# mfkiwl/msckf_stereo_c

Hardware: AMD Instinct MI355X
Metric: stereo frames/sec/node on EuRoC-shape input; ATE RMSE vs CPU ref (higher is better)
Workload: dtype f64

## Files before the change

### msckf_stereo_c_amd/csrc/hip/fe_kernels.hip

```cpp
#include <stdlib.h>
#include <mutex>
#include "fe_device.h"

__device__ __forceinline__ int reflect101(int i, int n) {
    if (n == 1) return 0;
    while (i < 0 || i >= n) { i = (i < 0) ? -i : 2 * (n - 1) - i; }
    return i;
}

#define P3_TW 16
#define P3_TH 8
struct Pyr3Job { const uint8_t *src; uint8_t *d1, *d2, *d3; int w0, h0; };

namespace {
constexpr int P3_R2H = 2 * P3_TH + 4, P3_R1H = 2 * P3_R2H + 4, P3_R0H = 2 * P3_R1H + 4;
constexpr int P3_P2W = 2 * P3_TW + 8, P3_P1W = 2 * (2 * P3_TW + 4) + 8;
constexpr int P3_P1S = P3_P1W + 8, P3_P2S = P3_P2W + 8;
typedef uint32_t __attribute__((aligned(1))) pd_u32u;

__device__ __forceinline__ uint2 pd_h4(uint32_t w0, uint32_t w1, uint32_t w2) {
    const int b0 = w0 & 255u, b1 = (w0 >> 8) & 255u, b2 = (w0 >> 16) & 255u, b3 = w0 >> 24, b4 = w1 & 255u, b5 = (w1 >> 8) & 255u,
              b6 = (w1 >> 16) & 255u, b7 = w1 >> 24, b8 = w2 & 255u, b9 = (w2 >> 8) & 255u, b10 = (w2 >> 16) & 255u;
    const uint32_t h0 = (uint32_t)(b0 + 4 * b1 + 6 * b2 + 4 * b3 + b4), h1 = (uint32_t)(b2 + 4 * b3 + 6 * b4 + 4 * b5 + b6);
    const uint32_t h2 = (uint32_t)(b4 + 4 * b5 + 6 * b6 + 4 * b7 + b8), h3 = (uint32_t)(b6 + 4 * b7 + 6 * b8 + 4 * b9 + b10);
    uint2 o; o.x = h0 | (h1 << 16); o.y = h2 | (h3 << 16);
    return o;
}
__device__ __forceinline__ uint32_t pd_v4(uint2 r0, uint2 r1, uint2 r2, uint2 r3, uint2 r4) {
    const uint32_t lo = (r0.x + r4.x) + 4u * (r1.x + r3.x) + 6u * r2.x + 0x00800080u;
    const uint32_t hi = (r0.y + r4.y) + 4u * (r1.y + r3.y) + 6u * r2.y + 0x00800080u;
    return ((lo >> 8) & 255u) | ((lo >> 24) << 8) | (((hi >> 8) & 255u) << 16) | ((hi >> 24) << 24);
}
__device__ __forceinline__ void pd_store4(uint8_t *row, int x, int w, uint32_t px) {
    if (x + 3 < w) *reinterpret_cast<pd_u32u *>(row + x) = px;
    else for (int k = 0; x + k < w; ++k) row[x + k] = (uint8_t)(px >> (8 * k));
}
__device__ __forceinline__ void pd_fill_halo(uint8_t *plane, int stride, int rows, int cols, int y_base, int x_base, int w, int h, int tid) {
    for (int i = tid; i < 4 * rows; i += 256) {
        const int r = i >> 2, q = i & 3;
        const int x = q < 2 ? q - 2 : w + q - 2, y = y_base + r;
        const int c = x - x_base;
        if (c < 0 || c >= cols || y < -2 || y > h + 1) continue;
        const int ys = reflect101(y, h) - y_base, xs = reflect101(x, w) - x_base;
        if (ys < 0 || ys >= rows || xs < 0 || xs >= cols) continue;
        plane[r * stride + 4 + c] = plane[ys * stride + 4 + xs];
    }
    for (int i = tid; i < 4 * cols; i += 256) {
        const int q = i / cols, c = i - q * cols;
        const int y = q < 2 ? q - 2 : h + q - 2, x = x_base + c;
        const int r = y - y_base;
        if (r < 0 || r >= rows || x < 0 || x >= w) continue;
        const int ys = reflect101(y, h) - y_base;
        if (ys < 0 || ys >= rows) continue;
        plane[r * stride + 4 + c] = plane[ys * stride + 4 + c];
    }
}
}

__global__ __launch_bounds__(256) void k_pyr_down3(const Pyr3Job *jobs, int n_jobs, int tiles_x, int tiles_y) {
    const int tiles = tiles_x * tiles_y;
    const int bx = blockIdx.x & 7, bq = blockIdx.x >> 3;
    const int ji = bx + 8 * (bq / tiles), tile = bq - (bq / tiles) * tiles;
    if (ji >= n_jobs) return;
    const Pyr3Job job = jobs[ji];
    const int w0 = job.w0, h0 = job.h0, w1 = (w0 + 1) >> 1, h1 = (h0 + 1) >> 1, w2 = (w1 + 1) >> 1, h2 = (h1 + 1) >> 1, w3 = (w2 + 1) >> 1, h3 = (h2 + 1) >> 1;
    const int ty = tile / tiles_x, tx = tile - ty * tiles_x;
    const int x3_0 = tx * P3_TW, y3_0 = ty * P3_TH;
    if (x3_0 >= w3 || y3_0 >= h3) return;
    __shared__ __attribute__((aligned(16))) uint16_t s_h0[P3_R0H][P3_P1W];
    __shared__ __attribute__((aligned(16))) uint8_t s_p1[P3_R1H][P3_P1S];
    __shared__ __attribute__((aligned(16))) uint16_t s_h1[P3_R1H][P3_P2W];
    __shared__ __attribute__((aligned(16))) uint8_t s_p2[P3_R2H][P3_P2S];
    __shared__ __attribute__((aligned(16))) uint16_t s_h2[P3_R2H][P3_TW];
    const int tid = threadIdx.x;
    const int x1b = 4 * x3_0 - 8, y1b = 4 * y3_0 - 6, y0b = 8 * y3_0 - 14;
    const int x2b = 2 * x3_0 - 4, y2b = 2 * y3_0 - 2;
    {
        const int pa = max(0, -y0b), pb = min(P3_R0H, h0 - y0b);
        constexpr int NG = P3_P1W / 4;
        int ga = (1 - x1b + 3) >> 2; ga = ga < 0 ? 0 : ga;
        int gb = min(min((w1 - 4 - x1b) >> 2, (w0 - 10 - 2 * x1b) >> 3) + 1, NG);
        if (w1 - 4 - x1b < 0 || w0 - 10 - 2 * x1b < 0) gb = 0;
        if (gb < ga) gb = ga;
        const int ng = gb - ga, n_fast = (pb - pa) * ng;
        const unsigned inv = ng > 0 ? (65536u + (unsigned)ng - 1u) / (unsigned)ng : 0u;
        constexpr int MAXIT = (P3_R0H * NG + 255) / 256;
        uint32_t la[MAXIT], lb[MAXIT], lc[MAXIT];
#pragma unroll
        for (int it = 0; it < MAXIT; ++it) {
            const int idx = tid + 256 * it;
            la[it] = lb[it] = lc[it] = 0u;
            if (idx < n_fast) {
                const int pr = (int)(((unsigned)idx * inv) >> 16), g = ga + idx - pr * ng, p = pa + pr;
                const uint8_t *q = job.src + (size_t)(y0b + p) * w0 + (2 * (x1b + 4 * g) - 2);
                la[it] = *reinterpret_cast<const pd_u32u *>(q); lb[it] = *reinterpret_cast<const pd_u32u *>(q + 4); lc[it] = *reinterpret_cast<const pd_u32u *>(q + 8);
            }
        }
#pragma unroll
        for (int it = 0; it < MAXIT; ++it) {
            const int idx = tid + 256 * it;
            if (idx < n_fast) {
                const int pr = (int)(((unsigned)idx * inv) >> 16), g = ga + idx - pr * ng, p = pa + pr;
                *reinterpret_cast<uint2 *>(&s_h0[p][4 * g]) = pd_h4(la[it], lb[it], lc[it]);
            }
        }
        const int n_edge = NG - ng, n_slow = (pb - pa) * n_edge;
        for (int idx = tid; idx < n_slow; idx += 256) {
            const int pr = idx / n_edge, e = idx - pr * n_edge, g = e < ga ? e : gb + (e - ga), p = pa + pr;
            const uint8_t *row = job.src + (size_t)(y0b + p) * w0;
#pragma unroll
            for (int j = 0; j < 4; ++j) {
                const int x1 = x1b + 4 * g + j;
                if (x1 < 0 || x1 >= w1) continue;
                const int c = 2 * x1;
                s_h0[p][4 * g + j] = (uint16_t)(row[reflect101(c - 2, w0)] + 4 * row[reflect101(c - 1, w0)] + 6 * row[reflect101(c, w0)] +
                                                4 * row[reflect101(c + 1, w0)] + row[reflect101(c + 2, w0)]);
            }
        }
    }
    __syncthreads();
    {
        const int ra = max(0, -y1b), rb = min(P3_R1H, h1 - y1b);
        constexpr int NG = P3_P1W / 4;
        const int n = (rb - ra) * NG;
        for (int idx = tid; idx < n; idx += 256) {
            const int rr = idx / NG, g = idx - rr * NG, r = ra + rr;
            const int y1 = y1b + r, x1 = x1b + 4 * g;
            if (x1 + 3 < 0 || x1 >= w1) continue;
            uint2 v[5];
#pragma unroll
            for (int k = 0; k < 5; ++k) {
                const int p = min(max(reflect101(2 * y1 - 2 + k, h0) - y0b, 0), P3_R0H - 1);
                v[k] = *reinterpret_cast<const uint2 *>(&s_h0[p][4 * g]);
            }
            const uint32_t px = pd_v4(v[0], v[1], v[2], v[3], v[4]);
            *reinterpret_cast<uint32_t *>(&s_p1[r][4 + 4 * g]) = px;
            if (r >= 6 && r < 6 + 4 * P3_TH && g >= 2 && g < 2 + P3_TW && x1 >= 0) pd_store4(job.d1 + (size_t)y1 * w1, x1, w1, px);
        }
    }
    __syncthreads();
    const bool edge1 = x1b < 0 || y1b < 0 || x1b + P3_P1W > w1 || y1b + P3_R1H > h1;
    if (edge1) { pd_fill_halo(&s_p1[0][0], P3_P1S, P3_R1H, P3_P1W, y1b, x1b, w1, h1, tid); __syncthreads(); }
    {
        constexpr int NG = P3_P2W / 4;
        const int ra = max(0, -2 - y1b), rb = min(P3_R1H, h1 + 2 - y1b);
        const int n = (rb - ra) * NG;
        for (int idx = tid; idx < n; idx += 256) {
            const int rr = idx / NG, g = idx - rr * NG, r = ra + rr;
            const uint32_t *q = reinterpret_cast<const uint32_t *>(&s_p1[r][8 * g]);
            const uint32_t d0 = q[0], d1 = q[1], d2 = q[2], d3 = q[3];
            *reinterpret_cast<uint2 *>(&s_h1[r][4 * g]) = pd_h4(__builtin_amdgcn_alignbyte(d1, d0, 2), __builtin_amdgcn_alignbyte(d2, d1, 2), __builtin_amdgcn_alignbyte(d3, d2, 2));
        }
    }
    __syncthreads();
    {
        constexpr int NG = P3_P2W / 4;
        const int ra = max(0, -y2b), rb = min(P3_R2H, h2 - y2b);
        const int n = (rb - ra) * NG;
        for (int idx = tid; idx < n; idx += 256) {
            const int rr = idx / NG, g = idx - rr * NG, r = ra + rr;
            const int y2 = y2b + r, x2 = x2b + 4 * g;
            if (x2 + 3 < 0 || x2 >= w2) continue;
            uint2 v[5];
#pragma unroll
            for (int k = 0; k < 5; ++k) v[k] = *reinterpret_cast<const uint2 *>(&s_h1[2 * r + k][4 * g]);
            const uint32_t px = pd_v4(v[0], v[1], v[2], v[3], v[4]);
            *reinterpret_cast<uint32_t *>(&s_p2[r][4 + 4 * g]) = px;
            if (r >= 2 && r < 2 + 2 * P3_TH && g >= 1 && g < 1 + P3_TW / 2 && x2 >= 0) pd_store4(job.d2 + (size_t)y2 * w2, x2, w2, px);
        }
    }
    __syncthreads();
    const bool edge2 = x2b < 0 || y2b < 0 || x2b + P3_P2W > w2 || y2b + P3_R2H > h2;
    if (edge2) { pd_fill_halo(&s_p2[0][0], P3_P2S, P3_R2H, P3_P2W, y2b, x2b, w2, h2, tid); __syncthreads(); }
    {
        constexpr int NG = P3_TW / 4;
        const int ra = max(0, -2 - y2b), rb = min(P3_R2H, h2 + 2 - y2b);
        const int n = (rb - ra) * NG;
        for (int idx = tid; idx < n; idx += 256) {
            const int rr = idx / NG, g = idx - rr * NG, r = ra + rr;
            const uint32_t *q = reinterpret_cast<const uint32_t *>(&s_p2[r][4 + 8 * g]);
            const uint32_t d0 = q[0], d1 = q[1], d2 = q[2], d3 = q[3];
            *reinterpret_cast<uint2 *>(&s_h2[r][4 * g]) = pd_h4(__builtin_amdgcn_alignbyte(d1, d0, 2), __builtin_amdgcn_alignbyte(d2, d1, 2), __builtin_amdgcn_alignbyte(d3, d2, 2));
        }
    }
    __syncthreads();
    {
        constexpr int NG = P3_TW / 4;
        const int rb = min(P3_TH, h3 - y3_0);
        const int n = rb * NG;
        for (int idx = tid; idx < n; idx += 256) {
            const int r = idx / NG, g = idx - r * NG;
            const int x3 = x3_0 + 4 * g;
            if (x3 >= w3) continue;
            uint2 v[5];
#pragma unroll
            for (int k = 0; k < 5; ++k) v[k] = *reinterpret_cast<const uint2 *>(&s_h2[2 * r + k][4 * g]);
            pd_store4(job.d3 + (size_t)(y3_0 + r) * w3, x3, w3, pd_v4(v[0], v[1], v[2], v[3], v[4]));
        }
    }
}

extern "C" void fe_launch_pyr_down3(const Pyr3Job *jobs_dev, int n_jobs, int max_w0, int max_h0, hipStream_t st) {
    const int w3 = (((max_w0 + 1) / 2 + 1) / 2 + 1) / 2, h3 = (((max_h0 + 1) / 2 + 1) / 2 + 1) / 2;
    const int tiles_x = (w3 + P3_TW - 1) / P3_TW, tiles_y = (h3 + P3_TH - 1) / P3_TH;
    hipLaunchKernelGGL(k_pyr_down3, dim3(8 * ((n_jobs + 7) / 8) * tiles_x * tiles_y), dim3(256), 0, st, jobs_dev, n_jobs, tiles_x, tiles_y);
}

#define DET_BORDER 8
#define DS_LANES 14
#define DS_COLS (4 * DS_LANES)

__device__ __forceinline__ unsigned long long det_key(unsigned int gen, int score, unsigned int order) {
    return ((unsigned long long)gen << 56) | ((unsigned long long)(unsigned int)score << 32) | (0xFFFFFFFFu - order);
}

__device__ __forceinline__ unsigned int isqrt48(unsigned long long v, double vd) {
    unsigned int r = (unsigned int)__builtin_amdgcn_sqrt(vd);
    while ((unsigned long long)r * r > v) --r;
    while ((unsigned long long)(r + 1) * (r + 1) <= v) ++r;
    return r;
}

template <int CTRL> __device__ __forceinline__ int det_dpp0(int v) { return __builtin_amdgcn_update_dpp(0, v, CTRL, 0xf, 0xf, true); }
template <int CTRL> __device__ __forceinline__ unsigned long long det_dpp0_64(unsigned long long v) {
    const unsigned int lo = (unsigned int)det_dpp0<CTRL>((int)(unsigned int)v), hi = (unsigned int)det_dpp0<CTRL>((int)(unsigned int)(v >> 32));
    return ((unsigned long long)hi << 32) | lo;
}

typedef short det_v2s __attribute__((ext_vector_type(2)));
__device__ __forceinline__ int det_dot2(int a, int b) { return __builtin_amdgcn_sdot2(__builtin_bit_cast(det_v2s, a), __builtin_bit_cast(det_v2s, b), 0, true); }
__device__ __forceinline__ int det_pksub(uint32_t a, uint32_t b) { return __builtin_bit_cast(int, (det_v2s)(__builtin_bit_cast(det_v2s, a) - __builtin_bit_cast(det_v2s, b))); }

__device__ __forceinline__ void det_hsum(int P01, int P23, int p0, int p2, int H[4]) {
    const int S = P01 + P23;
    H[0] = S + det_dpp0<0x101>(S);
    H[2] = H[0] + (det_dpp0<0x102>(P01) - P01);
    H[1] = H[0] + (det_dpp0<0x102>(p0) - p0);
    H[3] = H[2] + (det_dpp0<0x102>(p2) - p2);
}

struct DetPix { uint32_t lo, hi; };

__device__ __forceinline__ void det_hrow(uint32_t up, DetPix mid, uint32_t dn, int Ha[4], int Hb[4], int Hc[4]) {
    const uint32_t rn = (uint32_t)det_dpp0<0x101>((int)mid.hi);
    const uint32_t m01 = __builtin_amdgcn_perm(mid.hi, mid.lo, 0x0c040c03u);
    const uint32_t m23 = __builtin_amdgcn_perm(0u, mid.hi, 0x0c020c01u);
    const uint32_t m45 = __builtin_amdgcn_perm(rn, mid.hi, 0x0c040c03u);
    const int D01 = det_pksub(m23, m01), D23 = det_pksub(m45, m23);
    const int E01 = det_pksub(__builtin_amdgcn_perm(0u, dn, 0x0c010c00u), __builtin_amdgcn_perm(0u, up, 0x0c010c00u));
    const int E23 = det_pksub(__builtin_amdgcn_perm(0u, dn, 0x0c030c02u), __builtin_amdgcn_perm(0u, up, 0x0c030c02u));
    const int D0 = D01 & 0xffff, D2 = D23 & 0xffff, E0 = E01 & 0xffff, E2 = E23 & 0xffff;
    det_hsum(det_dot2(D01, D01), det_dot2(D23, D23), det_dot2(D0, D01), det_dot2(D2, D23), Ha);
    det_hsum(det_dot2(D01, E01), det_dot2(D23, E23), det_dot2(D0, E01), det_dot2(D2, E23), Hb);
    det_hsum(det_dot2(E01, E01), det_dot2(E23, E23), det_dot2(E0, E01), det_dot2(E2, E23), Hc);
}

__global__ __launch_bounds__(64) void k_detect_cells(const FeStreamDev *streams, int n_streams, int strips, int seg_rows, int waves, unsigned int gen) {
    const int xcd = blockIdx.x & 7, qb = blockIdx.x >> 3;
    const int si = xcd + 8 * (qb / waves), wi = qb - (qb / waves) * waves;
    if (si >= n_streams) return;
    const FeStreamDev &S = streams[si];
    const int W = S.curr0.w[0], H = S.curr0.h[0];
    const int cw = S.cell_w, ch = S.cell_h, det_cols = S.det_cols, det_floor = S.det_floor;
    unsigned long long *const cell_keys = S.cell_keys;
    const int lane = threadIdx.x, r = lane & 15;
    const int job = 4 * wi + (lane >> 4);
    const int seg = job / strips, strip = job - seg * strips;
    const int xs = DET_BORDER + DS_COLS * strip;
    const int ys = DET_BORDER + seg_rows * seg;
    const int y_end = min(ys + seg_rows, H - DET_BORDER);
    const bool job_on = xs < W - DET_BORDER && ys < y_end;
    if (!__any(job_on)) return;
    const int c0 = xs - 4 + 4 * r;
    const int cl = min(c0, W - 4);
    const uint8_t *img = S.curr0.lvl[0];
    typedef uint32_t __attribute__((aligned(1))) u32u;
    auto load = [&](int row) -> DetPix {
        const uint8_t *p = img + (size_t)min(max(row, 0), H - 1) * W + cl;
        DetPix v; v.lo = *(const u32u *)(p - 4); v.hi = *(const u32u *)p; return v;
    };
    int xin[4], cx[4];
    bool col_ok[4];
#pragma unroll
    for (int j = 0; j < 4; ++j) {
        const int x = c0 + 4 + j;
        cx[j] = x / cw; xin[j] = x - cx[j] * cw;
        col_ok[j] = job_on && r < DS_LANES && x < W - DET_BORDER;
    }
    int Va[4] = {0, 0, 0, 0}, Vb[4] = {0, 0, 0, 0}, Vc[4] = {0, 0, 0, 0};
    int pr = ys - 4;
    DetPix e_mid = load(pr), e_dn = load(pr + 1), e_nx = load(pr + 2);
    uint32_t e_up = load(pr - 1).hi;
#pragma unroll 1
    for (int k = 0; k < 7; ++k) {
        const DetPix nx = load(pr + 3);
        int Ha[4], Hb[4], Hc[4];
        det_hrow(e_up, e_mid, e_dn.hi, Ha, Hb, Hc);
#pragma unroll
        for (int j = 0; j < 4; ++j) { Va[j] += Ha[j]; Vb[j] += Hb[j]; Vc[j] += Hc[j]; }
        e_up = e_mid.hi; e_mid = e_dn; e_dn = e_nx; e_nx = nx; ++pr;
    }
    uint32_t l_up = load(ys - 5).hi;
    DetPix l_mid = load(ys - 4), l_dn = load(ys - 3), l_nx = load(ys - 2);
    int cy = ys / ch, yin = ys - cy * ch;
    int bs[4] = {0, 0, 0, 0};
    unsigned long long bk[4] = {0ULL, 0ULL, 0ULL, 0ULL};
    const int n_rows = seg_rows;
#pragma unroll 1
    for (int k = 0; k < n_rows; ++k) {
        const int y = ys + k;
        const bool row_ok = y < y_end;
        const DetPix enx = load(pr + 3), lnx = load(y - 1);
        {
            int Ha[4], Hb[4], Hc[4];
            det_hrow(e_up, e_mid, e_dn.hi, Ha, Hb, Hc);
#pragma unroll
            for (int j = 0; j < 4; ++j) { Va[j] += Ha[j]; Vb[j] += Hb[j]; Vc[j] += Hc[j]; }
            e_up = e_mid.hi; e_mid = e_dn; e_dn = e_nx; e_nx = enx; ++pr;
        }
#pragma unroll
        for (int j = 0; j < 4; ++j) {
            if (!(col_ok[j] && row_ok)) continue;
            const int a = Va[j], b = Vb[j], d = Vc[j];
            const int X = (a + d) - max(det_floor, bs[j]);
            if (X <= 0) continue;
            const int df = a - d;
            if (abs(df) >= X || 2 * abs(b) >= X) continue;
            const double discd = (double)df * (double)df + 4.0 * ((double)b * (double)b);
            if (discd >= (double)X * (double)X) continue;
            const long long disc = (long long)df * df + 4LL * ((long long)b * b);
            const int score = (a + d) - (int)isqrt48((unsigned long long)disc, discd);
            bs[j] = score;
            bk[j] = det_key(gen, score, (unsigned int)(yin * cw + xin[j]));
        }
        {
            int Ha[4], Hb[4], Hc[4];
            det_hrow(l_up, l_mid, l_dn.hi, Ha, Hb, Hc);
#pragma unroll
            for (int j = 0; j < 4; ++j) { Va[j] -= Ha[j]; Vb[j] -= Hb[j]; Vc[j] -= Hc[j]; }
            l_up = l_mid.hi; l_mid = l_dn; l_dn = l_nx; l_nx = lnx;
        }
        ++yin;
        const bool flush = job_on && row_ok && (yin == ch || y + 1 == y_end);
        if (cw < 4) {
            if (flush) {
#pragma unroll
                for (int j = 0; j < 4; ++j) {
                    if (bk[j]) atomicMax(&cell_keys[cy * det_cols + cx[j]], bk[j]);
                    bs[j] = 0; bk[j] = 0ULL;
                }
            }
        } else if (__any(flush)) {
            unsigned long long ka = 0ULL, kb = 0ULL;
#pragma unroll
            for (int j = 0; j < 4; ++j) {
                const unsigned long long v = flush ? bk[j] : 0ULL;
                if (cx[j] == cx[0]) ka = v > ka ? v : ka; else kb = v > kb ? v : kb;
            }
            const bool two = cx[3] != cx[0];
#pragma unroll 1
            for (int pass = 0; pass < 2; ++pass) {
                unsigned long long kk = pass ? kb : ka;
                const int id = flush ? (pass ? (two ? cx[3] : -1 - r) : cx[0]) : -1 - r;
                if (pass && !__any(flush && two)) break;
                {
                    const int o = det_dpp0<0x101>(id + 0x40000000) - 0x40000000; const unsigned long long v = det_dpp0_64<0x101>(kk);
                    if (o == id && v > kk) kk = v;
                }
                {
                    const int o = det_dpp0<0x102>(id + 0x40000000) - 0x40000000; const unsigned long long v = det_dpp0_64<0x102>(kk);
                    if (o == id && v > kk) kk = v;
                }
                {
                    const int o = det_dpp0<0x104>(id + 0x40000000) - 0x40000000; const unsigned long long v = det_dpp0_64<0x104>(kk);
                    if (o == id && v > kk) kk = v;
                }
                {
                    const int o = det_dpp0<0x108>(id + 0x40000000) - 0x40000000; const unsigned long long v = det_dpp0_64<0x108>(kk);
                    if (o == id && v > kk) kk = v;
                }
                const int left = det_dpp0<0x111>(id + 0x40000000) - 0x40000000;
                if (id >= 0 && left != id && kk) atomicMax(&cell_keys[cy * det_cols + id], kk);
            }
            if (flush) {
#pragma unroll
                for (int j = 0; j < 4; ++j) { bs[j] = 0; bk[j] = 0ULL; }
            }
        }
        if (yin == ch) { yin = 0; ++cy; }
    }
}

extern "C" void fe_launch_detect(const FeStreamDev *streams_dev, int n_streams, int max_w, int max_h, unsigned int gen, hipStream_t st) {
    const int strips = (max_w - 2 * DET_BORDER + DS_COLS - 1) / DS_COLS, rows = max_h - 2 * DET_BORDER;
    if (strips <= 0 || rows <= 0) return;
    int seg_rows = 32;
    while (seg_rows < 128 && (long long)n_streams * strips * ((rows + seg_rows - 1) / seg_rows) / 4 > 32768) seg_rows *= 2;
    const int segs = (rows + seg_rows - 1) / seg_rows;
    const int waves = (strips * segs + 3) / 4;
    hipLaunchKernelGGL(k_detect_cells, dim3(8 * ((n_streams + 7) / 8) * waves), dim3(64), 0, st, streams_dev, n_streams, strips, seg_rows, waves, gen);
}


__device__ __forceinline__ double det_atan(double x) {
    const bool inv = x > 1.0;
    if (inv) x = 1.0 / x;
    double c = 0.0, ac = 0.0;
    if (x > 0.875)      { c = 1.0;  ac = 0.78539816339744830962; }
    else if (x > 0.625) { c = 0.75; ac = 0.64350110879328438680; }
    else if (x > 0.375) { c = 0.5;  ac = 0.46364760900080611621; }
    else if (x > 0.125) { c = 0.25; ac = 0.24497866312686415417; }
    const double z = (x - c) / (1.0 + x * c);
    const double z2 = z * z;
    double p = 1.0 / 21.0;
    p = 1.0 / 19.0 - z2 * p;
    p = 1.0 / 17.0 - z2 * p;
    p = 1.0 / 15.0 - z2 * p;
    p = 1.0 / 13.0 - z2 * p;
    p = 1.0 / 11.0 - z2 * p;
    p = 1.0 / 9.0 - z2 * p;
    p = 1.0 / 7.0 - z2 * p;
    p = 1.0 / 5.0 - z2 * p;
    p = 1.0 / 3.0 - z2 * p;
    p = 1.0 - z2 * p;
    const double a = ac + z * p;
    return inv ? 1.5707963267948966192 - a : a;
}
__device__ __forceinline__ double det_tan(double t) {
    const bool inv = t > 0.78539816339744830962;
    if (inv) t = 1.5707963267948966192 - t;
    const double t2 = t * t;
    double s = 1.0 / 121645100408832000.0;
    s = 1.0 / 355687428096000.0 - t2 * s;
    s = 1.0 / 1307674368000.0 - t2 * s;
    s = 1.0 / 6227020800.0 - t2 * s;
    s = 1.0 / 39916800.0 - t2 * s;
    s = 1.0 / 362880.0 - t2 * s;
    s = 1.0 / 5040.0 - t2 * s;
    s = 1.0 / 120.0 - t2 * s;
    s = 1.0 / 6.0 - t2 * s;
    s = t * (1.0 - t2 * s);
    double c = 1.0 / 6402373705728000.0;
    c = 1.0 / 20922789888000.0 - t2 * c;
    c = 1.0 / 87178291200.0 - t2 * c;
    c = 1.0 / 479001600.0 - t2 * c;
    c = 1.0 / 3628800.0 - t2 * c;
    c = 1.0 / 40320.0 - t2 * c;
    c = 1.0 / 720.0 - t2 * c;
    c = 1.0 / 24.0 - t2 * c;
    c = 0.5 - t2 * c;
    c = 1.0 - t2 * c;
    return inv ? c / s : s / c;
}


__device__ __forceinline__ void undistort_pt(const CamDev &cam, const double *R, float u, float v, float &xo, float &yo) {
    const double fx = cam.K[0], fy = cam.K[1], cx = cam.K[2], cy = cam.K[3];
    double x = ((double)u - cx) / fx, y = ((double)v - cy) / fy;
    if (cam.model == MSKF_MODEL_EQUIDISTANT) {
        const double *k = cam.D;
        double theta_d = sqrt(x * x + y * y);
        const double half_pi = 1.5707963267948966;
        theta_d = theta_d > half_pi ? half_pi : (theta_d < -half_pi ? -half_pi : theta_d);
        double scale = 0.0;
        if (theta_d > 1e-8) {
            double theta = theta_d;
            for (int j = 0; j < 10; ++j) {
                const double t2 = theta * theta, t4 = t2 * t2, t6 = t4 * t2, t8 = t6 * t2;
                const double k0t2 = k[0] * t2, k1t4 = k[1] * t4, k2t6 = k[2] * t6, k3t8 = k[3] * t8;
                const double fix = (theta * (1 + k0t2 + k1t4 + k2t6 + k3t8) - theta_d) /
                                   (1 + 3 * k0t2 + 5 * k1t4 + 7 * k2t6 + 9 * k3t8);
                theta = theta - fix;
                if (fabs(fix) < 1e-8) break;
            }
            scale = det_tan(theta) / theta_d;
        }
        x = x * scale; y = y * scale;
    } else {
        const double k1 = cam.D[0], k2 = cam.D[1], p1 = cam.D[2], p2 = cam.D[3];
        const double x0 = x, y0 = y;
        for (int j = 0; j < 5; ++j) {
            const double r2 = x * x + y * y;
            const double icdist = 1.0 / (1.0 + (k2 * r2 + k1) * r2);
            const double deltaX = 2.0 * p1 * x * y + p2 * (r2 + 2.0 * x * x);
            const double deltaY = p1 * (r2 + 2.0 * y * y) + 2.0 * p2 * x * y;
            x = (x0 - deltaX) * icdist;
            y = (y0 - deltaY) * icdist;
        }
    }
    if (R) {
        const double X = R[0] * x + R[1] * y + R[2];
        const double Y = R[3] * x + R[4] * y + R[5];
        const double Wd = R[6] * x + R[7] * y + R[8];
        x = X / Wd; y = Y / Wd;
    } else {
        x = x / 1.0; y = y / 1.0;
    }
    xo = (float)(x * 1.0 + 0.0);
    yo = (float)(y * 1.0 + 0.0);
}

__device__ __forceinline__ void distort_pt(const CamDev &cam, float xf, float yf, float &uo, float &vo) {
    const double fx = cam.K[0], fy = cam.K[1], cx = cam.K[2], cy = cam.K[3];
    const double x = (double)xf, y = (double)yf;
    double xd, yd;
    if (cam.model == MSKF_MODEL_EQUIDISTANT) {
        const double *k = cam.D;
        const double r = sqrt(x * x + y * y);
        const double theta = det_atan(r);
        const double t2 = theta * theta, t4 = t2 * t2, t6 = t4 * t2, t8 = t4 * t4;
        const double theta_d = theta * (1 + k[0] * t2 + k[1] * t4 + k[2] * t6 + k[3] * t8);
        const double scale = (r > 1e-8) ? theta_d / r : 1.0;
        xd = x * scale; yd = y * scale;
    } else {
        const double k1 = cam.D[0], k2 = cam.D[1], p1 = cam.D[2], p2 = cam.D[3];
        const double r2 = x * x + y * y, r4 = r2 * r2;
        const double a1 = 2.0 * x * y, a2 = r2 + 2.0 * x * x, a3 = r2 + 2.0 * y * y;
        const double cdist = 1.0 + k1 * r2 + k2 * r4;
        xd = x * cdist + p1 * a1 + p2 * a2;
        yd = y * cdist + p1 * a3 + p2 * a1;
    }
    uo = (float)(xd * fx + cx);
    vo = (float)(yd * fy + cy);
}

#define LK_HALF 7
#define LK_WIN 15
#define LK_ITERS 30

template <int CTRL> __device__ __forceinline__ int dpp_add(int v) {
    return v + __builtin_amdgcn_update_dpp(0, v, CTRL, 0xf, 0xf, false);
}
__device__ __forceinline__ double lk_scaled_f64(long long b) {
    return __longlong_as_double(b + 0x41F8000000000000LL) - 6442450944.0;
}

typedef short l4_v2s __attribute__((ext_vector_type(2)));
#define L4_DW 6
#define L4_TROWS 18
#define L4_SROWS 20
#define L4_MAXOX 8
#define L4_MAXOY (L4_SROWS - 16)

typedef unsigned short l4_v2u __attribute__((ext_vector_type(2)));
template <int KA, int KC> __device__ __forceinline__ int l4_mad24_k(int x) {
    int d;
    asm("v_mad_i32_i24 %0, %1, %2, %3" : "=v"(d) : "n"(KA), "v"(x), "n"(KC));
    return d;
}
template <int KA> __device__ __forceinline__ int l4_mad24_kv(int x, int c) {
    int d;
    asm("v_mad_i32_i24 %0, %1, %2, %3" : "=v"(d) : "n"(KA), "v"(x), "v"(c));
    return d;
}
__device__ __forceinline__ int l4_mad24(int a, int b, int c) {
    int d;
    asm("v_mad_i32_i24 %0, %1, %2, %3" : "=v"(d) : "v"(a), "v"(b), "s"(c));
    return d;
}
__device__ __forceinline__ int l4_mad24_vvv(int a, int b, int c) {
    int d;
    asm("v_mad_i32_i24 %0, %1, %2, %3" : "=v"(d) : "v"(a), "v"(b), "v"(c));
    return d;
}
__device__ __forceinline__ int l4_dot2(int pair, int w, int acc) {
    return __builtin_amdgcn_sdot2(__builtin_bit_cast(l4_v2s, pair), __builtin_bit_cast(l4_v2s, w), acc, false);
}
__device__ __forceinline__ int l4_dot2k(int pair, int w, int k) {
    return __builtin_amdgcn_sdot2(__builtin_bit_cast(l4_v2s, pair), __builtin_bit_cast(l4_v2s, w), k, true);
}
__device__ __forceinline__ int l4_pack_shr9(int a, int b) {
    const l4_v2u v = __builtin_bit_cast(l4_v2u, __builtin_amdgcn_perm((uint32_t)b, (uint32_t)a, 0x06050201u));
    return __builtin_bit_cast(int, (l4_v2u)(v >> (unsigned short)1));
}
#define L4_SHL1 0x101
#define L4_SHR1 0x111
template <int CTRL> __device__ __forceinline__ int l4_dpp0(int v) {
    return __builtin_amdgcn_update_dpp(0, v, CTRL, 0xf, 0xf, true);
}
__device__ __forceinline__ long long l4_row_sum(int v) {
    v = dpp_add<0xB1>(v);
    v = dpp_add<0x4E>(v);
    long long s = (long long)v;
    {
        const int lo = __builtin_amdgcn_update_dpp(0, (int)s, 0x141, 0xf, 0xf, true), hi = __builtin_amdgcn_update_dpp(0, (int)(s >> 32), 0x141, 0xf, 0xf, true);
        s += (long long)(((unsigned long long)(unsigned int)hi << 32) | (unsigned int)lo);
    }
    {
        const int lo = __builtin_amdgcn_update_dpp(0, (int)s, 0x140, 0xf, 0xf, true), hi = __builtin_amdgcn_update_dpp(0, (int)(s >> 32), 0x140, 0xf, 0xf, true);
        s += (long long)(((unsigned long long)(unsigned int)hi << 32) | (unsigned int)lo);
    }
    return s;
}

struct __attribute__((packed, aligned(4))) l4_u4 { uint32_t v[4]; };
struct __attribute__((packed, aligned(4))) l4_u2 { uint32_t v[2]; };
template <int ROWS>
__device__ __forceinline__ void l4_stage(const uint8_t *img, int w, int h, int x0, int y0, uint32_t *dst, int r, bool on) {
    const bool fast = x0 >= 0 && y0 >= 0 && x0 + 4 * L4_DW <= w && y0 + ROWS <= h;
    if (fast) {
        if (on) {
            const uint8_t *p = img + l4_mad24_vvv(y0 + r, w, x0);
            const l4_u4 a = *(const l4_u4 *)p;
            const l4_u2 b = *(const l4_u2 *)(p + 16);
            uint32_t *d = dst + L4_DW * r;
            d[0] = a.v[0]; d[1] = a.v[1]; d[2] = a.v[2]; d[3] = a.v[3]; d[4] = b.v[0]; d[5] = b.v[1];
            if (r < ROWS - 16) {
                const uint8_t *p2 = img + l4_mad24_vvv(y0 + 16 + r, w, x0);
                const l4_u4 a2 = *(const l4_u4 *)p2;
                const l4_u2 b2 = *(const l4_u2 *)(p2 + 16);
                uint32_t *d2 = dst + L4_DW * (16 + r);
                d2[0] = a2.v[0]; d2[1] = a2.v[1]; d2[2] = a2.v[2]; d2[3] = a2.v[3]; d2[4] = b2.v[0]; d2[5] = b2.v[1];
            }
        }
        return;
    }
    constexpr int N = ROWS * L4_DW, PER = (N + 15) / 16;
    typedef uint32_t __attribute__((aligned(1))) l4_u32u;
    uint32_t v[PER];
#pragma unroll
    for (int i = 0; i < PER; ++i) {
        const int e = r + 16 * i;
        v[i] = 0;
        if (on && e < N) {
            const int row = (e * 43) >> 8, c = e - L4_DW * row;
            const uint8_t *rp = img + l4_mad24_vvv(min(max(y0 + row, 0), h - 1), w, 0);
            const int xb = x0 + 4 * c, xc = min(max(xb, 0), w - 4), sh = xb - xc;
            const uint32_t D = *(const l4_u32u *)(rp + xc);
            const uint32_t first = (D & 255u) * 0x01010101u, last = (D >> 24) * 0x01010101u;
            v[i] = sh < 0 ? first : sh >= 4 ? last : __builtin_amdgcn_alignbyte(last, D, (uint32_t)sh);
        }
    }
#pragma unroll
    for (int i = 0; i < PER; ++i) { const int e = r + 16 * i; if (on && e < N) dst[e] = v[i]; }
}

template <int K> __device__ __forceinline__ int l4_pair(const uint32_t *a) {
    constexpr int q = K >> 2, m = K & 3;
    if (m == 0) return (int)__builtin_amdgcn_perm(0u, a[q], 0x0c010c00u);
    if (m == 1) return (int)__builtin_amdgcn_perm(0u, a[q], 0x0c020c01u);
    if (m == 2) return (int)__builtin_amdgcn_perm(0u, a[q], 0x0c030c02u);
    return (int)__builtin_amdgcn_perm(a[q + 1], a[q], 0x0c040c03u);
// ... 589 lines not shown
```

Baseline: 99510.

## Rewrite 3-level pyramid downsample as register-streaming wave kernel; fuse detector window update

The 3-level pyramid kernel is replaced. The old version was a 256-thread shared-memory tiled kernel with several barriers. The new version is a 64-lane wavefront kernel: each lane owns a level-3 column, streams source rows vertically through rolling registers, and gets horizontal neighbours through DPP lane shifts, byte perms and udot4 filter taps. Reflect-101 borders are handled by precomputed per-lane perm selectors, and the launcher sizes row segments to keep enough waves in flight. The corner detector now folds the add-new-row and subtract-old-row products into one horizontal sum per row, and primes the window with 8 rows instead of 7. Both changes aim to cut LDS traffic, barriers and ALU work, at the cost of intricate border logic and a detector window reordering that could shift results.

New measurement: 107,200, median of 6. +7.7%, better.

```diff
diff --git a/msckf_stereo_c_amd/csrc/hip/fe_kernels.hip b/msckf_stereo_c_amd/csrc/hip/fe_kernels.hip
--- a/msckf_stereo_c_amd/csrc/hip/fe_kernels.hip
+++ b/msckf_stereo_c_amd/csrc/hip/fe_kernels.hip
@@ -8,202 +8,162 @@
     return i;
 }
 
-#define P3_TW 16
-#define P3_TH 8
+#define P3_HALO 2
+#define P3_OWN 12
+#define P3_SEG_ROWS 8
 struct Pyr3Job { const uint8_t *src; uint8_t *d1, *d2, *d3; int w0, h0; };
 
 namespace {
-constexpr int P3_R2H = 2 * P3_TH + 4, P3_R1H = 2 * P3_R2H + 4, P3_R0H = 2 * P3_R1H + 4;
-constexpr int P3_P2W = 2 * P3_TW + 8, P3_P1W = 2 * (2 * P3_TW + 4) + 8;
-constexpr int P3_P1S = P3_P1W + 8, P3_P2S = P3_P2W + 8;
 typedef uint32_t __attribute__((aligned(1))) pd_u32u;
-
-__device__ __forceinline__ uint2 pd_h4(uint32_t w0, uint32_t w1, uint32_t w2) {
-    const int b0 = w0 & 255u, b1 = (w0 >> 8) & 255u, b2 = (w0 >> 16) & 255u, b3 = w0 >> 24, b4 = w1 & 255u, b5 = (w1 >> 8) & 255u,
-              b6 = (w1 >> 16) & 255u, b7 = w1 >> 24, b8 = w2 & 255u, b9 = (w2 >> 8) & 255u, b10 = (w2 >> 16) & 255u;
-    const uint32_t h0 = (uint32_t)(b0 + 4 * b1 + 6 * b2 + 4 * b3 + b4), h1 = (uint32_t)(b2 + 4 * b3 + 6 * b4 + 4 * b5 + b6);
-    const uint32_t h2 = (uint32_t)(b4 + 4 * b5 + 6 * b6 + 4 * b7 + b8), h3 = (uint32_t)(b6 + 4 * b7 + 6 * b8 + 4 * b9 + b10);
+typedef uint16_t __attribute__((aligned(1))) pd_u16u;
+typedef unsigned long long __attribute__((aligned(1))) pd_u64u;
+typedef const __attribute__((address_space(1))) pd_u64u *pd_gld64;
+typedef __attribute__((address_space(1))) pd_u32u *pd_gst32;
+typedef __attribute__((address_space(1))) pd_u16u *pd_gst16;
+typedef __attribute__((address_space(1))) uint8_t *pd_gst8;
+
+template <int CTRL> __device__ __forceinline__ uint32_t pd_dpp0(uint32_t v) { return (uint32_t)__builtin_amdgcn_update_dpp(0, (int)v, CTRL, 0xf, 0xf, true); }
+__device__ __forceinline__ uint32_t pd_dot4(uint32_t a, uint32_t b, uint32_t c) { return __builtin_amdgcn_udot4(a, b, c, false); }
+
+__device__ __forceinline__ uint2 pd_h4(uint32_t e0, uint32_t e1, uint32_t e2) {
+    const uint32_t h0 = pd_dot4(e0, 0x04060401u, e1 & 255u), h1 = pd_dot4(e0, 0x04010000u, pd_dot4(e1, 0x00010406u, 0u));
+    const uint32_t h2 = pd_dot4(e1, 0x04060401u, e2 & 255u), h3 = pd_dot4(e1, 0x04010000u, pd_dot4(e2, 0x00010406u, 0u));
     uint2 o; o.x = h0 | (h1 << 16); o.y = h2 | (h3 << 16);
     return o;
 }
-__device__ __forceinline__ uint32_t pd_v4(uint2 r0, uint2 r1, uint2 r2, uint2 r3, uint2 r4) {
-    const uint32_t lo = (r0.x + r4.x) + 4u * (r1.x + r3.x) + 6u * r2.x + 0x00800080u;
-    const uint32_t hi = (r0.y + r4.y) + 4u * (r1.y + r3.y) + 6u * r2.y + 0x00800080u;
-    return ((lo >> 8) & 255u) | ((lo >> 24) << 8) | (((hi >> 8) & 255u) << 16) | ((hi >> 24) << 24);
-}
-__device__ __forceinline__ void pd_store4(uint8_t *row, int x, int w, uint32_t px) {
-    if (x + 3 < w) *reinterpret_cast<pd_u32u *>(row + x) = px;
-    else for (int k = 0; x + k < w; ++k) row[x + k] = (uint8_t)(px >> (8 * k));
-}
-__device__ __forceinline__ void pd_fill_halo(uint8_t *plane, int stride, int rows, int cols, int y_base, int x_base, int w, int h, int tid) {
-    for (int i = tid; i < 4 * rows; i += 256) {
-        const int r = i >> 2, q = i & 3;
-        const int x = q < 2 ? q - 2 : w + q - 2, y = y_base + r;
-        const int c = x - x_base;
-        if (c < 0 || c >= cols || y < -2 || y > h + 1) continue;
-        const int ys = reflect101(y, h) - y_base, xs = reflect101(x, w) - x_base;
-        if (ys < 0 || ys >= rows || xs < 0 || xs >= cols) continue;
-        plane[r * stride + 4 + c] = plane[ys * stride + 4 + xs];
-    }
-    for (int i = tid; i < 4 * cols; i += 256) {
-        const int q = i / cols, c = i - q * cols;
-        const int y = q < 2 ? q - 2 : h + q - 2, x = x_base + c;
-        const int r = y - y_base;
-        if (r < 0 || r >= rows || x < 0 || x >= w) continue;
-        const int ys = reflect101(y, h) - y_base;
-        if (ys < 0 || ys >= rows) continue;
-        plane[r * stride + 4 + c] = plane[ys * stride + 4 + c];
-    }
-}
-}
-
-__global__ __launch_bounds__(256) void k_pyr_down3(const Pyr3Job *jobs, int n_jobs, int tiles_x, int tiles_y) {
-    const int tiles = tiles_x * tiles_y;
-    const int bx = blockIdx.x & 7, bq = blockIdx.x >> 3;
-    const int ji = bx + 8 * (bq / tiles), tile = bq - (bq / tiles) * tiles;
+__device__ __forceinline__ uint32_t pd_v2(uint32_t r0, uint32_t r1, uint32_t r2, uint32_t r3, uint32_t r4) {
+    return (r0 + r4 + 0x00800080u) + ((r1 + r2 + r3) << 2) + (r2 << 1);
+}
+__device__ __forceinline__ void pd_store4(uint8_t *lvl, uint32_t off, int n, uint32_t px) {
+    if (n >= 4) { *(pd_gst32)(lvl + off) = px; return; }
+    *(pd_gst8)(lvl + off) = (uint8_t)px;
+    if (n >= 2) *(pd_gst8)(lvl + off + 1u) = (uint8_t)(px >> 8);
+    if (n >= 3) *(pd_gst8)(lvl + off + 2u) = (uint8_t)(px >> 16);
+}
+__device__ uint32_t pd_fix_sel(int cb, int w, int p0, int base, uint32_t ident) {
+    uint32_t sel = 0u;
+    for (int b = 0; b < 4; ++b) {
+        const int col = cb - 2 + p0 + b;
+        uint32_t s = (ident >> (8 * b)) & 255u;
+        if (col < 0 || col >= w) {
+            const int sp = reflect101(col, w) - cb + 2 - base;
+            if (sp >= 0 && sp < 8) s = (uint32_t)sp;
+        }
+        sel |= s << (8 * b);
+    }
+    return sel;
+}
+__device__ __forceinline__ void pd_vfix(uint32_t &a, uint32_t &b, uint32_t c, uint32_t &d, uint32_t &e, int yd, int hs) {
+    if (2 * yd + 1 == hs) { e = hs == 1 ? c : a; d = hs == 1 ? c : b; }
+    else if (2 * yd + 2 == hs) e = c;
+    if (yd == 0) { a = e; b = d; }
+}
+}
+
+__global__ __launch_bounds__(64) void k_pyr_down3(const Pyr3Job *jobs, int n_jobs, int strips, int seg3, int waves) {
+    const int xcd = blockIdx.x & 7, qb = blockIdx.x >> 3;
+    const int ji = xcd + 8 * (qb / waves), wi = qb - (qb / waves) * waves;
     if (ji >= n_jobs) return;
     const Pyr3Job job = jobs[ji];
     const int w0 = job.w0, h0 = job.h0, w1 = (w0 + 1) >> 1, h1 = (h0 + 1) >> 1, w2 = (w1 + 1) >> 1, h2 = (h1 + 1) >> 1, w3 = (w2 + 1) >> 1, h3 = (h2 + 1) >> 1;
-    const int ty = tile / tiles_x, tx = tile - ty * tiles_x;
-    const int x3_0 = tx * P3_TW, y3_0 = ty * P3_TH;
-    if (x3_0 >= w3 || y3_0 >= h3) return;
-    __shared__ __attribute__((aligned(16))) uint16_t s_h0[P3_R0H][P3_P1W];
-    __shared__ __attribute__((aligned(16))) uint8_t s_p1[P3_R1H][P3_P1S];
-    __shared__ __attribute__((aligned(16))) uint16_t s_h1[P3_R1H][P3_P2W];
-    __shared__ __attribute__((aligned(16))) uint8_t s_p2[P3_R2H][P3_P2S];
-    __shared__ __attribute__((aligned(16))) uint16_t s_h2[P3_R2H][P3_TW];
-    const int tid = threadIdx.x;
-    const int x1b = 4 * x3_0 - 8, y1b = 4 * y3_0 - 6, y0b = 8 * y3_0 - 14;
-    const int x2b = 2 * x3_0 - 4, y2b = 2 * y3_0 - 2;
-    {
-        const int pa = max(0, -y0b), pb = min(P3_R0H, h0 - y0b);
-        constexpr int NG = P3_P1W / 4;
-        int ga = (1 - x1b + 3) >> 2; ga = ga < 0 ? 0 : ga;
-        int gb = min(min((w1 - 4 - x1b) >> 2, (w0 - 10 - 2 * x1b) >> 3) + 1, NG);
-        if (w1 - 4 - x1b < 0 || w0 - 10 - 2 * x1b < 0) gb = 0;
-        if (gb < ga) gb = ga;
-        const int ng = gb - ga, n_fast = (pb - pa) * ng;
-        const unsigned inv = ng > 0 ? (65536u + (unsigned)ng - 1u) / (unsigned)ng : 0u;
-        constexpr int MAXIT = (P3_R0H * NG + 255) / 256;
-        uint32_t la[MAXIT], lb[MAXIT], lc[MAXIT];
-#pragma unroll
-        for (int it = 0; it < MAXIT; ++it) {
-            const int idx = tid + 256 * it;
-            la[it] = lb[it] = lc[it] = 0u;
-            if (idx < n_fast) {
-                const int pr = (int)(((unsigned)idx * inv) >> 16), g = ga + idx - pr * ng, p = pa + pr;
-                const uint8_t *q = job.src + (size_t)(y0b + p) * w0 + (2 * (x1b + 4 * g) - 2);
-                la[it] = *reinterpret_cast<const pd_u32u *>(q); lb[it] = *reinterpret_cast<const pd_u32u *>(q + 4); lc[it] = *reinterpret_cast<const pd_u32u *>(q + 8);
-            }
-        }
-#pragma unroll
-        for (int it = 0; it < MAXIT; ++it) {
-            const int idx = tid + 256 * it;
-            if (idx < n_fast) {
-                const int pr = (int)(((unsigned)idx * inv) >> 16), g = ga + idx - pr * ng, p = pa + pr;
-                *reinterpret_cast<uint2 *>(&s_h0[p][4 * g]) = pd_h4(la[it], lb[it], lc[it]);
-            }
-        }
-        const int n_edge = NG - ng, n_slow = (pb - pa) * n_edge;
-        for (int idx = tid; idx < n_slow; idx += 256) {
-            const int pr = idx / n_edge, e = idx - pr * n_edge, g = e < ga ? e : gb + (e - ga), p = pa + pr;
-            const uint8_t *row = job.src + (size_t)(y0b + p) * w0;
-#pragma unroll
-            for (int j = 0; j < 4; ++j) {
-                const int x1 = x1b + 4 * g + j;
-                if (x1 < 0 || x1 >= w1) continue;
-                const int c = 2 * x1;
-                s_h0[p][4 * g + j] = (uint16_t)(row[reflect101(c - 2, w0)] + 4 * row[reflect101(c - 1, w0)] + 6 * row[reflect101(c, w0)] +
-                                                4 * row[reflect101(c + 1, w0)] + row[reflect101(c + 2, w0)]);
-            }
-        }
-    }
-    __syncthreads();
-    {
-        const int ra = max(0, -y1b), rb = min(P3_R1H, h1 - y1b);
-        constexpr int NG = P3_P1W / 4;
-        const int n = (rb - ra) * NG;
-        for (int idx = tid; idx < n; idx += 256) {
-            const int rr = idx / NG, g = idx - rr * NG, r = ra + rr;
-            const int y1 = y1b + r, x1 = x1b + 4 * g;
-            if (x1 + 3 < 0 || x1 >= w1) continue;
-            uint2 v[5];
-#pragma unroll
-            for (int k = 0; k < 5; ++k) {
-                const int p = min(max(reflect101(2 * y1 - 2 + k, h0) - y0b, 0), P3_R0H - 1);
-                v[k] = *reinterpret_cast<const uint2 *>(&s_h0[p][4 * g]);
-            }
-            const uint32_t px = pd_v4(v[0], v[1], v[2], v[3], v[4]);
-            *reinterpret_cast<uint32_t *>(&s_p1[r][4 + 4 * g]) = px;
-            if (r >= 6 && r < 6 + 4 * P3_TH && g >= 2 && g < 2 + P3_TW && x1 >= 0) pd_store4(job.d1 + (size_t)y1 * w1, x1, w1, px);
-        }
-    }
-    __syncthreads();
-    const bool edge1 = x1b < 0 || y1b < 0 || x1b + P3_P1W > w1 || y1b + P3_R1H > h1;
-    if (edge1) { pd_fill_halo(&s_p1[0][0], P3_P1S, P3_R1H, P3_P1W, y1b, x1b, w1, h1, tid); __syncthreads(); }
-    {
-        constexpr int NG = P3_P2W / 4;
-        const int ra = max(0, -2 - y1b), rb = min(P3_R1H, h1 + 2 - y1b);
-        const int n = (rb - ra) * NG;
-        for (int idx = tid; idx < n; idx += 256) {
-            const int rr = idx / NG, g = idx - rr * NG, r = ra + rr;
-            const uint32_t *q = reinterpret_cast<const uint32_t *>(&s_p1[r][8 * g]);
-            const uint32_t d0 = q[0], d1 = q[1], d2 = q[2], d3 = q[3];
-            *reinterpret_cast<uint2 *>(&s_h1[r][4 * g]) = pd_h4(__builtin_amdgcn_alignbyte(d1, d0, 2), __builtin_amdgcn_alignbyte(d2, d1, 2), __builtin_amdgcn_alignbyte(d3, d2, 2));
-        }
-    }
-    __syncthreads();
-    {
-        constexpr int NG = P3_P2W / 4;
-        const int ra = max(0, -y2b), rb = min(P3_R2H, h2 - y2b);
-        const int n = (rb - ra) * NG;
-        for (int idx = tid; idx < n; idx += 256) {
-            const int rr = idx / NG, g = idx - rr * NG, r = ra + rr;
-            const int y2 = y2b + r, x2 = x2b + 4 * g;
-            if (x2 + 3 < 0 || x2 >= w2) continue;
-            uint2 v[5];
-#pragma unroll
-            for (int k = 0; k < 5; ++k) v[k] = *reinterpret_cast<const uint2 *>(&s_h1[2 * r + k][4 * g]);
-            const uint32_t px = pd_v4(v[0], v[1], v[2], v[3], v[4]);
-            *reinterpret_cast<uint32_t *>(&s_p2[r][4 + 4 * g]) = px;
-            if (r >= 2 && r < 2 + 2 * P3_TH && g >= 1 && g < 1 + P3_TW / 2 && x2 >= 0) pd_store4(job.d2 + (size_t)y2 * w2, x2, w2, px);
-        }
-    }
-    __syncthreads();
-    const bool edge2 = x2b < 0 || y2b < 0 || x2b + P3_P2W > w2 || y2b + P3_R2H > h2;
-    if (edge2) { pd_fill_halo(&s_p2[0][0], P3_P2S, P3_R2H, P3_P2W, y2b, x2b, w2, h2, tid); __syncthreads(); }
-    {
-        constexpr int NG = P3_TW / 4;
-        const int ra = max(0, -2 - y2b), rb = min(P3_R2H, h2 + 2 - y2b);
-        const int n = (rb - ra) * NG;
-        for (int idx = tid; idx < n; idx += 256) {
-            const int rr = idx / NG, g = idx - rr * NG, r = ra + rr;
-            const uint32_t *q = reinterpret_cast<const uint32_t *>(&s_p2[r][4 + 8 * g]);
-            const uint32_t d0 = q[0], d1 = q[1], d2 = q[2], d3 = q[3];
-            *reinterpret_cast<uint2 *>(&s_h2[r][4 * g]) = pd_h4(__builtin_amdgcn_alignbyte(d1, d0, 2), __builtin_amdgcn_alignbyte(d2, d1, 2), __builtin_amdgcn_alignbyte(d3, d2, 2));
-        }
-    }
-    __syncthreads();
-    {
-        constexpr int NG = P3_TW / 4;
-        const int rb = min(P3_TH, h3 - y3_0);
-        const int n = rb * NG;
-        for (int idx = tid; idx < n; idx += 256) {
-            const int r = idx / NG, g = idx - r * NG;
-            const int x3 = x3_0 + 4 * g;
-            if (x3 >= w3) continue;
-            uint2 v[5];
-#pragma unroll
-            for (int k = 0; k < 5; ++k) v[k] = *reinterpret_cast<const uint2 *>(&s_h2[2 * r + k][4 * g]);
-            pd_store4(job.d3 + (size_t)(y3_0 + r) * w3, x3, w3, pd_v4(v[0], v[1], v[2], v[3], v[4]));
+    const int lane = threadIdx.x, r = lane & 15;
+    const int sj = 4 * wi + (lane >> 4);
+    const int seg = sj / strips, strip = sj - seg * strips;
+    const int x3 = P3_OWN * strip - P3_HALO + r;
+    const int y3a = seg3 * seg, y3b = min(y3a + seg3, h3);
+    const bool job_on = P3_OWN * strip < w3 && y3a < h3;
+    if (!__any(job_on)) return;
+    const bool own = job_on && r >= P3_HALO && r < P3_HALO + P3_OWN && x3 < w3;
+    uint32_t sa0 = 0x03020100u, sa1 = 0x07060504u, sa2 = 0x07060504u, sb0 = 0x03020100u, sb1 = 0x07060504u, sc0 = 0x03020100u, sc1 = 0x07060504u;
+    if (x3 >= 0 && 8 * x3 < w0 && (x3 == 0 || 8 * x3 + 8 >= w0 || 4 * x3 + 4 >= w1 || 2 * x3 + 2 >= w2)) {
+        sa0 = pd_fix_sel(8 * x3, w0, 0, 0, sa0); sa1 = pd_fix_sel(8 * x3, w0, 4, 0, sa1); sa2 = pd_fix_sel(8 * x3, w0, 8, 4, sa2);
+        sb0 = pd_fix_sel(4 * x3, w1, 0, 0, sb0); sb1 = pd_fix_sel(4 * x3, w1, 4, 0, sb1);
+        sc0 = pd_fix_sel(2 * x3, w2, 0, 0, sc0); sc1 = pd_fix_sel(2 * x3, w2, 4, 0, sc1);
+    }
+    const int c0 = min(max(8 * x3, 0), w0 - 1), cl = max(min(c0, w0 - 8), 0);
+    const int sh0 = 8 * (c0 - cl), k0 = 2 * (h0 - 1);
+    const uint32_t last8 = (uint32_t)max(w0 * h0 - 8, 0);
+    auto load = [&](int s) -> uint2 {
+        int y = max(s, -s);
+        y = max(min(y, k0 - y), 0);
+        const uint32_t a = (uint32_t)y * (uint32_t)w0 + (uint32_t)cl, ac = min(a, last8);
+        const int sh = sh0 + 8 * (int)(a - ac);
+        const unsigned long long q = *(pd_gld64)(job.src + ac) >> sh;
+        uint2 o; o.x = (uint32_t)q; o.y = (uint32_t)(q >> 32);
+        return o;
+    };
+    uint2 R0[5];
+    uint32_t R1[5], R2[5];
+#pragma unroll
+    for (int k = 0; k < 5; ++k) { R0[k].x = R0[k].y = 0u; R1[k] = R2[k] = 0u; }
+    int t = y3a - 2;
+    uint2 q[4];
+#pragma unroll
+    for (int k = 0; k < 4; ++k) q[k] = load(8 * t + k);
+    const int y1a = 4 * y3a, y1b = min(4 * (y3a + seg3), h1), y2a = 2 * y3a, y2b = min(2 * (y3a + seg3), h2);
+    const int n1 = own ? min(w1 - 4 * x3, 4) : 0, n2 = own ? min(w2 - 2 * x3, 2) : 0;
+#pragma unroll 1
+    for (int it = 0; it < seg3 + 3; ++it, ++t) {
+#pragma unroll
+        for (int p = 0; p < 8; ++p) {
+            const uint2 px = q[p & 3];
+            q[p & 3] = load(8 * t + p + 4);
+            const uint32_t lf = pd_dpp0<0x111>(px.y), rt = pd_dpp0<0x101>(px.x);
+            const uint32_t e0 = __builtin_amdgcn_alignbyte(px.x, lf, 2), e1 = __builtin_amdgcn_alignbyte(px.y, px.x, 2), e2 = __builtin_amdgcn_alignbyte(rt, px.y, 2);
+#pragma unroll
+            for (int k = 0; k < 4; ++k) R0[k] = R0[k + 1];
+            R0[4] = pd_h4(__builtin_amdgcn_perm(e1, e0, sa0), __builtin_amdgcn_perm(e1, e0, sa1), __builtin_amdgcn_perm(e2, e1, sa2));
+            if (p & 1) continue;
+            const int y1 = 4 * t + p / 2 - 1;
+            const uint32_t p1 = __builtin_amdgcn_perm(pd_v2(R0[0].y, R0[1].y, R0[2].y, R0[3].y, R0[4].y), pd_v2(R0[0].x, R0[1].x, R0[2].x, R0[3].x, R0[4].x), 0x07050301u);
+            if (n1 > 0 && y1 >= y1a && y1 < y1b) pd_store4(job.d1, (uint32_t)(y1 * w1 + 4 * x3), n1, p1);
+            {
+                const uint32_t l1 = pd_dpp0<0x111>(p1), r1 = pd_dpp0<0x101>(p1);
+                const uint32_t u0 = __builtin_amdgcn_alignbyte(p1, l1, 2), u1 = __builtin_amdgcn_alignbyte(r1, p1, 2);
+                const uint32_t g0 = __builtin_amdgcn_perm(u1, u0, sb0), g1 = __builtin_amdgcn_perm(u1, u0, sb1);
+#pragma unroll
+                for (int k = 0; k < 4; ++k) R1[k] = R1[k + 1];
+                R1[4] = pd_dot4(g0, 0x04060401u, g1 & 255u) | (pd_dot4(g0, 0x04010000u, pd_dot4(g1, 0x00010406u, 0u)) << 16);
+            }
+            if (p != 2 && p != 6) continue;
+            const int y2 = 2 * t - 1 + (p == 6);
+            uint32_t p2;
+            {
+                uint32_t a = R1[0], b = R1[1], d = R1[3], e = R1[4];
+                pd_vfix(a, b, R1[2], d, e, y2, h1);
+                p2 = __builtin_amdgcn_perm(0u, pd_v2(a, b, R1[2], d, e), 0x0c0c0301u);
+            }
+            if (n2 > 0 && y2 >= y2a && y2 < y2b) {
+                const uint32_t o = (uint32_t)(y2 * w2 + 2 * x3);
+                if (n2 == 2) *(pd_gst16)(job.d2 + o) = (uint16_t)p2; else *(pd_gst8)(job.d2 + o) = (uint8_t)p2;
+            }
+            {
+                const uint32_t l2 = pd_dpp0<0x111>(p2), r2 = pd_dpp0<0x101>(p2);
+                const uint32_t u0 = __builtin_amdgcn_perm(p2, l2, 0x05040100u);
+                const uint32_t g0 = __builtin_amdgcn_perm(r2, u0, sc0), g1 = __builtin_amdgcn_perm(r2, u0, sc1);
+#pragma unroll
+                for (int k = 0; k < 4; ++k) R2[k] = R2[k + 1];
+                R2[4] = pd_dot4(g0, 0x04060401u, g1 & 255u);
+            }
+            if (p != 6) continue;
+            const int y3 = t - 1;
+            uint32_t a = R2[0], b = R2[1], d = R2[3], e = R2[4];
+            pd_vfix(a, b, R2[2], d, e, y3, h2);
+            const uint32_t p3 = (((a + e) + 4u * (b + d) + 6u * R2[2] + 128u) >> 8) & 255u;
+            if (own && y3 >= y3a && y3 < y3b) *(pd_gst8)(job.d3 + (uint32_t)(y3 * w3 + x3)) = (uint8_t)p3;
         }
     }
 }
 
 extern "C" void fe_launch_pyr_down3(const Pyr3Job *jobs_dev, int n_jobs, int max_w0, int max_h0, hipStream_t st) {
     const int w3 = (((max_w0 + 1) / 2 + 1) / 2 + 1) / 2, h3 = (((max_h0 + 1) / 2 + 1) / 2 + 1) / 2;
-    const int tiles_x = (w3 + P3_TW - 1) / P3_TW, tiles_y = (h3 + P3_TH - 1) / P3_TH;
-    hipLaunchKernelGGL(k_pyr_down3, dim3(8 * ((n_jobs + 7) / 8) * tiles_x * tiles_y), dim3(256), 0, st, jobs_dev, n_jobs, tiles_x, tiles_y);
+    if (n_jobs <= 0 || w3 <= 0 || h3 <= 0) return;
+    const int strips = (w3 + P3_OWN - 1) / P3_OWN;
+    int target = P3_SEG_ROWS;
+    while (target > 4 && (long long)n_jobs * strips * ((h3 + target - 1) / target) / 4 < 2048) target /= 2;
+    const int segs = (h3 + target - 1) / target, seg3 = (h3 + segs - 1) / segs;
+    const int waves = (strips * segs + 3) / 4;
+    hipLaunchKernelGGL(k_pyr_down3, dim3(8 * ((n_jobs + 7) / 8) * waves), dim3(64), 0, st, jobs_dev, n_jobs, strips, seg3, waves);
 }
 
 #define DET_BORDER 8
@@ -241,7 +201,7 @@
 
 struct DetPix { uint32_t lo, hi; };
 
-__device__ __forceinline__ void det_hrow(uint32_t up, DetPix mid, uint32_t dn, int Ha[4], int Hb[4], int Hc[4]) {
+__device__ __forceinline__ void det_prod(uint32_t up, DetPix mid, uint32_t dn, int P[12]) {
     const uint32_t rn = (uint32_t)det_dpp0<0x101>((int)mid.hi);
     const uint32_t m01 = __builtin_amdgcn_perm(mid.hi, mid.lo, 0x0c040c03u);
     const uint32_t m23 = __builtin_amdgcn_perm(0u, mid.hi, 0x0c020c01u);
@@ -250,9 +210,15 @@
     const int E01 = det_pksub(__builtin_amdgcn_perm(0u, dn, 0x0c010c00u), __builtin_amdgcn_perm(0u, up, 0x0c010c00u));
     const int E23 = det_pksub(__builtin_amdgcn_perm(0u, dn, 0x0c030c02u), __builtin_amdgcn_perm(0u, up, 0x0c030c02u));
     const int D0 = D01 & 0xffff, D2 = D23 & 0xffff, E0 = E01 & 0xffff, E2 = E23 & 0xffff;
-    det_hsum(det_dot2(D01, D01), det_dot2(D23, D23), det_dot2(D0, D01), det_dot2(D2, D23), Ha);
-    det_hsum(det_dot2(D01, E01), det_dot2(D23, E23), det_dot2(D0, E01), det_dot2(D2, E23), Hb);
-    det_hsum(det_dot2(E01, E01), det_dot2(E23, E23), det_dot2(E0, E01), det_dot2(E2, E23), Hc);
+    P[0] = det_dot2(D01, D01); P[1] = det_dot2(D23, D23); P[2] = det_dot2(D0, D01); P[3] = det_dot2(D2, D23);
+    P[4] = det_dot2(D01, E01); P[5] = det_dot2(D23, E23); P[6] = det_dot2(D0, E01); P[7] = det_dot2(D2, E23);
+    P[8] = det_dot2(E01, E01); P[9] = det_dot2(E23, E23); P[10] = det_dot2(E0, E01); P[11] = det_dot2(E2, E23);
+}
+__device__ __forceinline__ void det_vadd(const int P[12], int Va[4], int Vb[4], int Vc[4]) {
+    int Ha[4], Hb[4], Hc[4];
+    det_hsum(P[0], P[1], P[2], P[3], Ha); det_hsum(P[4], P[5], P[6], P[7], Hb); det_hsum(P[8], P[9], P[10], P[11], Hc);
+#pragma unroll
+    for (int j = 0; j < 4; ++j) { Va[j] += Ha[j]; Vb[j] += Hb[j]; Vc[j] += Hc[j]; }
 }
 
 __global__ __launch_bounds__(64) void k_detect_cells(const FeStreamDev *streams, int n_streams, int strips, int seg_rows, int waves, unsigned int gen) {
@@ -292,12 +258,11 @@
     DetPix e_mid = load(pr), e_dn = load(pr + 1), e_nx = load(pr + 2);
     uint32_t e_up = load(pr - 1).hi;
 #pragma unroll 1
-    for (int k = 0; k < 7; ++k) {
+    for (int k = 0; k < 8; ++k) {
         const DetPix nx = load(pr + 3);
-        int Ha[4], Hb[4], Hc[4];
-        det_hrow(e_up, e_mid, e_dn.hi, Ha, Hb, Hc);
-#pragma unroll
-        for (int j = 0; j < 4; ++j) { Va[j] += Ha[j]; Vb[j] += Hb[j]; Vc[j] += Hc[j]; }
+        int P[12];
+        det_prod(e_up, e_mid, e_dn.hi, P);
+        det_vadd(P, Va, Vb, Vc);
         e_up = e_mid.hi; e_mid = e_dn; e_dn = e_nx; e_nx = nx; ++pr;
     }
     uint32_t l_up = load(ys - 5).hi;
@@ -311,13 +276,6 @@
         const int y = ys + k;
         const bool row_ok = y < y_end;
         const DetPix enx = load(pr + 3), lnx = load(y - 1);
-        {
-            int Ha[4], Hb[4], Hc[4];
-            det_hrow(e_up, e_mid, e_dn.hi, Ha, Hb, Hc);
-#pragma unroll
-            for (int j = 0; j < 4; ++j) { Va[j] += Ha[j]; Vb[j] += Hb[j]; Vc[j] += Hc[j]; }
-            e_up = e_mid.hi; e_mid = e_dn; e_dn = e_nx; e_nx = enx; ++pr;
-        }
 #pragma unroll
         for (int j = 0; j < 4; ++j) {
             if (!(col_ok[j] && row_ok)) continue;
@@ -334,10 +292,13 @@
             bk[j] = det_key(gen, score, (unsigned int)(yin * cw + xin[j]));
         }
         {
-            int Ha[4], Hb[4], Hc[4];
-            det_hrow(l_up, l_mid, l_dn.hi, Ha, Hb, Hc);
-#pragma unroll
-            for (int j = 0; j < 4; ++j) { Va[j] -= Ha[j]; Vb[j] -= Hb[j]; Vc[j] -= Hc[j]; }
+            int Pe[12], Pl[12];
+            det_prod(e_up, e_mid, e_dn.hi, Pe);
+            det_prod(l_up, l_mid, l_dn.hi, Pl);
+#pragma unroll
+            for (int j = 0; j < 12; ++j) Pe[j] -= Pl[j];
+            det_vadd(Pe, Va, Vb, Vc);
+            e_up = e_mid.hi; e_mid = e_dn; e_dn = e_nx; e_nx = enx; ++pr;
             l_up = l_mid.hi; l_mid = l_dn; l_dn = l_nx; l_nx = lnx;
         }
         ++yin;
```
